# google/neural-light-transport

Hardware: AMD Instinct MI355X
Metric: rendered Mtexels/s at 1024^2 UV (full Model.call forward: U-Net + UV->camera warp); at N > 1: N collective-free replicas of this forward (weak scaling).  The data-parallel TRAIN step with the RCCL gradient all-reduce (BASELINE config 4) is `train_step`: value = Mtexels/s over all ranks, speedup_vs_o (higher is better)
Workload: dtype f32 via 3xbf16 split, 9 exact products, fp32 accumulate (the LDS-tiled encoder convs: fp32 operands as three bf16 terms on v_mfma_f32_16x16x32_bf16, every term product exact in fp32); f32 storage everywhere, every other launch native f32; 1 GPU; BASELINE config 3: dragon_specular relight+view-synth, depth0 16/depth 256, 4 frames/GPU, 1024^2 UV, k=4 obs maps, 512^2 camera warp; frames_per_gpu=4, uv=1024, k=4, cam=512, conv_algo=auto, plan=fused ends, launch=eager, two HIP streams, distinct_batches_rotated=3, launch_tape_replays=0, parallelism=dp1 (frames sharded, no forward collective), world=1, dist_world_size=1, device=cuda:0

## Files before the change

include/nlt_hip.h:

```cpp
#ifndef NLT_HIP_H_
#define NLT_HIP_H_

#ifdef __cplusplus
extern "C" {
#endif

typedef enum {
  NLT_OK = 0,
  NLT_ERR_BAD_ARG = -1,
  NLT_ERR_UNSUPPORTED = -2,
  NLT_ERR_LAUNCH = -3
} nlt_status;

typedef enum {
  NLT_CONV1X1 = 0,
  NLT_CONV_K2S2 = 1,
  NLT_CONV_K2S1 = 2,
  NLT_DECONV_K2S2 = 3,
  NLT_DECONV_K2S1 = 4,
  NLT_CONV_K3S1 = 5,
  NLT_CONV_K3S2 = 6,
  NLT_DECONV_K3S1 = 7,
  NLT_DECONV_K3S2 = 8
} nlt_conv_mode;
// ... 361 lines not shown
int nlt_conv_wino_forward(int mode, const float* src, int ld, int cin, int frames, int kobs, int h, int w,
                          const float* packed, const float* bias, int cout, int tn,
                          float* out, int ldo, float* mean_out, int ldm, int act, float alpha, void* stream);
int nlt_pack_conv_wino_weights_adjoint(int adj_mode, const float* w_keras, int cpre, int cout, int tn, int full, int lo,
                                       float* packed, void* stream);
int nlt_conv_wino_backward_data(int adj_mode, const float* dpre, int ldp, int cpre, int n, int h, int w,
                                const float* packed, int cout, int tn, float* out, int ldo,
                                const float* mask_src, int ldm, float mask_alpha, int accumulate, void* stream);

int nlt_conv_c32_supported(int mode, int cin, int cout);
int nlt_conv_c32_forward(int mode, const float* src, int ld, int cin, int frames, int kobs, int h, int w,
                         const float* packed, const float* bias, int cout,
                         float* out, int ldo, float* mean_out, int ldm, int act, float alpha, void* stream);

long nlt_conv_tile_packed_floats(int mode, int cin, int cout, int tn);
int nlt_pack_conv_tile_weights(int mode, const float* w_keras, int cin, int cout, int tn, float* packed, void* stream);
int nlt_conv_tile_forward(int mode, const float* src, int ld, int cin, int frames, int kobs, int h, int w,
                          const float* packed, const float* bias, int cout, int tn,
                          float* out, int ldo, float* mean_out, int ldm, int act, float alpha, void* stream);

int nlt_pack_conv_tile_weights_adjoint(int adj_mode, const float* w_keras, int cpre, int cout, int tn, int full, int lo,
                                       float* packed, void* stream);
int nlt_conv_tile_backward_data(int adj_mode, const float* dpre, int ldp, int cpre, int n, int h, int w,
                                const float* packed, int cout, int tn, float* out, int ldo,
                                const float* mask_src, int ldm, float mask_alpha, int accumulate,
                                int split_c, const float* split_y, float* split_d, float split_alpha, int split_partial,
                                void* stream);

long nlt_conv_tile3_packed_elems(int mode, int cin, int cout, int tn);
int nlt_pack_conv_tile3_weights(int mode, const float* w_keras, int cin, int cout, int tn, unsigned short* packed, void* stream);
int nlt_conv_tile3_forward(int mode, int nprod, const float* src, int ld, int cin, int frames, int kobs, int h, int w,
                           const unsigned short* packed, const float* bias, int cout, int tn,
                           float* out, int ldo, float* mean_out, int ldm, int act, float alpha, void* stream);

long nlt_chmix_bf16_packed_elems(int cin, int cout);
int nlt_chmix_bf16_pack(const float* w_keras, int cin, int cout, unsigned short* packed, void* stream);
int nlt_chmix_bf16_forward(const unsigned short* x, long texels, int cin, const unsigned short* packed,
                           const float* bias, int cout, int act, float alpha, unsigned short* out, void* stream);

int nlt_conv_k3_forward(int mode, int algo, const float* x, int n, int h, int w, int cin,
                        const float* w_keras, const float* bias, int cout, float* y,
                        int act, float alpha, void* stream);

int nlt_conv_k3_backward_data(int mode, int algo, const float* dpre, int n, int h, int w, int cin,
                              const float* w_keras, int cout, float* dx, void* stream);

long nlt_conv_k3_wgrad_workspace_floats(int mode, int n, int h, int w, int cin, int cout);
int nlt_conv_k3_backward_weights(int mode, const float* x, int n, int h, int w, int cin,
                                 const float* dpre, int cout, float* dw_keras, float* dbias,
                                 float* workspace, long workspace_floats, void* stream);

#ifdef __cplusplus
}
#endif
#endif
```

neural-light-transport_amd/_capi.py:

```python
import ctypes
import threading
import os

import torch

_HERE = os.path.dirname(os.path.abspath(__file__))
LIB_PATH = os.environ.get('NLT_HIP_LIB') or os.path.join(_HERE, 'libnlt_hip.so')

CONV1X1, CONV_K2S2, CONV_K2S1, DECONV_K2S2, DECONV_K2S1 = range(5)
CONV_K3S1, CONV_K3S2, DECONV_K3S1, DECONV_K3S2 = range(5, 9)
ALGO_AUTO, ALGO_DIRECT, ALGO_MFMA = range(3)

_c_int, _c_long, _c_float, _vp = ctypes.c_int, ctypes.c_long, ctypes.c_float, ctypes.c_void_p
_c_double = ctypes.c_double
MAP_F64, MAP_F32, MAP_F16 = range(3)

SIGNATURES = {
    'nlt_version': (ctypes.c_char_p, []),
    'nlt_status_string': (ctypes.c_char_p, [_c_int]),
    'nlt_packed_weight_floats': (_c_long, [_c_int] * 4),
    'nlt_pack_conv_weights': (_c_int, [_c_int, _vp, _c_int, _c_int, _c_int, _vp, _vp]),
    'nlt_conv_forward': (_c_int, [_c_int, _c_int, _c_int, _vp, _c_int, _c_int, _vp, _c_int, _c_int,
                                  _c_int, _c_int, _c_int, _vp, _vp, _vp, _c_int, _vp, _c_int,
                                  _c_int, _c_float, _vp, _c_int, _c_int, _vp]),
# ... 74 lines not shown
    'nlt_conv_forward_splitk': (_c_int, [_c_int, _c_int, _c_int, _vp, _vp, _c_int, _c_int, _vp, _c_int, _c_int,
                                         _c_int, _c_int, _c_int, _vp, _vp, _c_int, _vp, _c_int, _c_int, _c_float,
                                         _vp, _c_int, _c_int, _vp]),
    'nlt_conv_forward_map': (_c_int, [_c_int, _c_int, _c_int, _vp, _vp, _c_int, _c_int, _vp, _c_int, _c_int,
                                      _c_int, _c_int, _c_int, _vp, _vp, _c_int, _vp, _c_int, _c_int, _c_float,
                                      _vp, _c_int, _vp]),
    'nlt_dec_block_forward_map': (_c_int, [_vp, _vp, _c_int, _c_int, _c_int, _c_int, _vp, _vp, _vp, _c_int, _c_float, _vp, _vp, _vp]),
    'nlt_back_forward_map': (_c_int, [_vp, _vp, _c_int, _vp, _c_int, _c_int, _c_int, _vp, _vp, _vp, _vp, _c_float, _vp, _vp, _vp]),
    'nlt_front_ovr_forward': (_c_int, [_vp] * 3 + [_c_int] * 3 + [_vp] * 5 + [_c_int, _c_float, _vp, _c_int, _vp, _vp, _vp]),
    'nlt_front_ovr_forward_u8': (_c_int, [_vp] * 4 + [_c_int] * 3 + [_vp] * 5 + [_c_int, _c_float, _vp, _c_int, _vp, _vp, _vp]),
    'nlt_conv_backward_data': (_c_int, [_c_int, _c_int, _c_int, _vp, _vp, _c_int, _c_int, _c_int, _c_int, _c_int, _vp, _vp, _c_int,
                                        _vp, _c_int, _vp, _c_int, _c_float, _c_int, _c_int, _vp, _vp, _c_float, _c_int, _vp]),
    'nlt_conv_tile_packed_floats': (_c_long, [_c_int] * 4),
    'nlt_pack_conv_tile_weights': (_c_int, [_c_int, _vp, _c_int, _c_int, _c_int, _vp, _vp]),
    'nlt_conv_tile_forward': (_c_int, [_c_int, _vp, _c_int, _c_int, _c_int, _c_int, _c_int, _c_int, _vp, _vp, _c_int, _c_int,
                                       _vp, _c_int, _vp, _c_int, _c_int, _c_float, _vp]),
    'nlt_pack_conv_tile_weights_adjoint': (_c_int, [_c_int, _vp, _c_int, _c_int, _c_int, _c_int, _c_int, _vp, _vp]),
    'nlt_conv_c32_supported': (_c_int, [_c_int] * 3),
    'nlt_conv_c32_forward': (_c_int, [_c_int, _vp, _c_int, _c_int, _c_int, _c_int, _c_int, _c_int, _vp, _vp, _c_int,
                                      _vp, _c_int, _vp, _c_int, _c_int, _c_float, _vp]),
    'nlt_conv_wino_packed_floats': (_c_long, [_c_int] * 4),
    'nlt_pack_conv_wino_weights': (_c_int, [_c_int, _vp, _c_int, _c_int, _c_int, _vp, _vp]),
    'nlt_conv_wino_forward': (_c_int, [_c_int, _vp, _c_int, _c_int, _c_int, _c_int, _c_int, _c_int, _vp, _vp, _c_int, _c_int,
                                       _vp, _c_int, _vp, _c_int, _c_int, _c_float, _vp]),
    'nlt_pack_conv_wino_weights_adjoint': (_c_int, [_c_int, _vp, _c_int, _c_int, _c_int, _c_int, _c_int, _vp, _vp]),
    'nlt_conv_wino_backward_data': (_c_int, [_c_int, _vp, _c_int, _c_int, _c_int, _c_int, _c_int, _vp, _c_int, _c_int, _vp, _c_int,
                                             _vp, _c_int, _c_float, _c_int, _vp]),
    'nlt_conv_tile_backward_data': (_c_int, [_c_int, _vp, _c_int, _c_int, _c_int, _c_int, _c_int, _vp, _c_int, _c_int, _vp, _c_int,
                                             _vp, _c_int, _c_float, _c_int, _c_int, _vp, _vp, _c_float, _c_int, _vp]),
    'nlt_conv_tile3_packed_elems': (_c_long, [_c_int] * 4),
    'nlt_pack_conv_tile3_weights': (_c_int, [_c_int, _vp, _c_int, _c_int, _c_int, _vp, _vp]),
    'nlt_conv_tile3_forward': (_c_int, [_c_int, _c_int, _vp, _c_int, _c_int, _c_int, _c_int, _c_int, _c_int, _vp, _vp, _c_int, _c_int,
                                        _vp, _c_int, _vp, _c_int, _c_int, _c_float, _vp]),
    'nlt_conv_bf16_packed_elems': (_c_long, [_c_int] * 4),
    'nlt_conv_bf16_pack': (_c_int, [_c_int, _vp, _c_int, _c_int, _c_int, _vp, _vp]),
    'nlt_conv_bf16_forward': (_c_int, [_c_int, _c_int, _vp, _c_int, _c_int, _c_int, _vp, _c_int, _c_int, _c_int,
                                       _c_int, _c_int, _c_int, _vp, _vp, _c_int, _vp, _c_int, _c_int, _c_int, _c_float, _vp]),
    'nlt_obs_mean_bf16': (_c_int, [_vp, _c_int, _c_int, _c_long, _c_int, _vp, _c_int, _vp]),
    'nlt_chmix_bf16_packed_elems': (_c_long, [_c_int, _c_int]),
    'nlt_chmix_bf16_pack': (_c_int, [_vp, _c_int, _c_int, _vp, _vp]),
    'nlt_chmix_bf16_forward': (_c_int, [_vp, _c_long, _c_int, _vp, _vp, _c_int, _c_int, _c_float, _vp, _vp]),
    'nlt_cosine_map': (_c_int, [_vp] * 4 + [_c_double] * 3 + [_c_long, _vp, _vp, _vp]),
    'nlt_albedo': (_c_int, [_vp, _c_int, _c_long, _vp, _vp, _vp]),
    'nlt_diffuse_base': (_c_int, [_vp, _vp, _c_int, _c_long, _vp, _vp]),
    'nlt_remap_bilinear_u8': (_c_int, [_vp, _c_int, _c_int, _c_int, _vp, _c_int, _c_int, _c_int, _c_int, _c_int, _vp, _vp]),
    'nlt_remap_bilinear_f32': (_c_int, [_vp, _c_int, _c_int, _c_int, _vp, _c_int, _c_int, _c_int, _c_int, _c_int, _vp, _vp]),
    'nlt_uv_index_map_workspace_bytes': (_c_long, [_c_int, _c_int, _c_long]),
    'nlt_uv_index_map': (_c_int, [_vp, _vp, _c_long, _c_int, _c_int, _c_int, _c_int, _c_double, _vp, _vp, _vp, _vp]),
    'nlt_knn_indices': (_c_int, [_vp, _c_int, _vp, _c_int, _c_int, _vp, _vp]),
    'nlt_psnr_sums': (_c_int, [_vp, _vp, _vp, _c_long, _c_int, _vp, _vp, _vp]),
    'nlt_gather_frames_u8': (_c_int, [_vp, _vp, _c_int, _c_long, _vp, _vp]),
    'nlt_assemble_batch': (_c_int, [_vp] * 6 + [_c_int, _c_int, _c_long, _c_int] + [_vp] * 6 + [_vp]),
    'nlt_warp_backward_det_workspace_bytes': (_c_long, [_c_int] * 5),
    'nlt_warp_backward_det': (_c_int, [_vp, _vp] + [_c_int] * 5 + [_vp, _vp, _c_long, _vp]),
    'nlt_resize_bilinear_backward_gather': (_c_int, [_vp] + [_c_int] * 6 + [_vp, _vp]),
    'nlt_loss_det_workspace_floats': (_c_long, [_c_int]),
    'nlt_l2_loss_forward_det': (_c_int, [_vp, _vp, _c_int, _c_long, _vp, _vp, _c_long, _vp]),
    'nlt_l2_loss_weighted_forward_det': (_c_int, [_vp, _vp, _vp, _c_int, _c_long, _c_int, _vp, _vp, _c_long, _vp]),
    'nlt_l2_train_loss_det': (_c_int, [_vp, _vp, _vp, _c_int, _c_long, _c_float, _vp, _vp, _vp, _vp, _c_long, _vp]),
    'nlt_barron_det_slots_floats': (_c_long, [_c_int] * 3),
    'nlt_barron_loss_det': (_c_int, [_vp, _vp, _c_int, _c_int, _c_int, _vp, _vp, _vp, _vp, _c_long, _vp]),
    'nlt_stem_backward_det_workspace_floats': (_c_long, [_c_int] * 4),
    'nlt_stem_backward_det': (_c_int, [_vp] * 6 + [_c_int] * 5 + [_vp] * 6 + [_vp, _c_long, _vp]),
    'nlt_head_backward_det_workspace_floats': (_c_long, [_c_int] * 5),
    'nlt_head_backward_det': (_c_int, [_vp, _c_int, _c_int, _vp, _c_int, _c_int, _vp, _vp, _c_int, _c_int, _c_int,
                                       _vp, _c_int, _vp, _c_int, _vp, _vp, _vp, _c_long, _vp]),
# ... 819 lines not shown


def pack_conv_wino_weights(mode, w_keras, cin, cout, tn, full=None, lo=0):
    src = (mode, _ptr(_dense(w_keras, 'w_keras')), cin, cout, tn)
    if full is None:
        name, args = 'nlt_pack_conv_wino_weights', src
    else:
        name, args = 'nlt_pack_conv_wino_weights_adjoint', src + (full, lo)
    return _pack('nlt_conv_wino_packed_floats', (mode, cin, cout, tn), name, args, torch.float32, w_keras.device)


def conv_wino_forward(mode, src, ld, cin, frames, kobs, h, w, packed, bias, cout, tn, out, ldo, mean_out, ldm, act=True, alpha=0.3):
    _call('nlt_conv_wino_forward', mode, _ptr(src), ld, cin, frames, kobs, h, w, _ptr(packed), _ptr(bias), cout, tn, _ptr(out), ldo,
          _ptr(mean_out), ldm, 1 if act else 0, float(alpha))


def conv_wino_backward_data(adj_mode, dpre, cpre, ldp, n, h, w, packed, cout, tn, out, ldo, mask_src=None, ldm=0, mask_alpha=0.3,
                            accumulate=False):
    _call('nlt_conv_wino_backward_data', adj_mode, _ptr(dpre), ldp, cpre, n, h, w, _ptr(packed), cout, tn, _ptr(out), ldo,
          _ptr(mask_src), ldm, float(mask_alpha), 1 if accumulate else 0)


def pack_conv_tile3_weights(mode, w_keras, cin, cout, tn):
    return _pack('nlt_conv_tile3_packed_elems', (mode, cin, cout, tn),
                 'nlt_pack_conv_tile3_weights', (mode, _ptr(_dense(w_keras, 'w_keras')), cin, cout, tn), torch.int16, w_keras.device)


def conv_tile3_forward(mode, src, ld, cin, frames, kobs, h, w, packed, bias, cout, tn, out, ldo, mean_out, ldm,
                       act=True, alpha=0.3, nprod=6):
    _call('nlt_conv_tile3_forward', mode, nprod, _ptr(src), ld, cin, frames, kobs, h, w, packed.data_ptr(), _ptr(bias), cout, tn,
          _ptr(out), ldo, _ptr(mean_out), ldm, 1 if act else 0, float(alpha))


def conv_bf16_pack(mode, w_keras, c0, c1, cout):
    return _pack('nlt_conv_bf16_packed_elems', (mode, c0, c1, cout),
                 'nlt_conv_bf16_pack', (mode, _ptr(_dense(w_keras, 'w_keras')), c0, c1, cout), torch.bfloat16, w_keras.device)


def _any_ptr(t, what):
    if t is None:
        return None, 0
    if not (t.is_cuda and t.dtype in (torch.float32, torch.bfloat16)):
        raise NLTError("%s: expected a float32 / bfloat16 CUDA tensor, got %s on %s" % (what, t.dtype, t.device))
    return t.data_ptr(), 1 if t.dtype == torch.float32 else 0


def conv_bf16_forward(mode, src0, c0, ld0, src1, c1, ld1, n, h, w, w_packed, bias, cout, out, ldo, act=True, alpha=0.3, tile_hint=0):
    p0, f0 = _any_ptr(src0, 'src0')
    p1, f1 = _any_ptr(src1, 'src1')
    po, fo = _any_ptr(out, 'out')
    _call('nlt_conv_bf16_forward', mode, tile_hint, p0, ld0, c0, f0, p1, ld1, c1, f1, n, h, w,
          _tptr(w_packed, torch.bfloat16, 'w_packed'), _ptr(bias), cout, po, ldo, fo, 1 if act else 0, float(alpha))


def obs_mean_bf16(obs, n, k, hw, c, out, ldo):
    if obs.dtype != torch.bfloat16 or out.dtype != torch.bfloat16:
        raise NLTError("obs_mean_bf16: bfloat16 tensors expected")
    _call('nlt_obs_mean_bf16', obs.data_ptr(), n, k, hw, c, out.data_ptr(), ldo)


def chmix_bf16_pack(w_keras):
    cin, cout = w_keras.shape[2], w_keras.shape[3]
    return _pack('nlt_chmix_bf16_packed_elems', (cin, cout),
                 'nlt_chmix_bf16_pack', (_ptr(_dense(w_keras, 'w_keras')), cin, cout), torch.bfloat16, w_keras.device)


# ... 245 lines not shown
```

neural-light-transport_amd/csrc/conv_tile3.hip:

```cpp
#include "nlt_common.h"
#include "pack_common.h"

namespace {

typedef __attribute__((ext_vector_type(8))) __bf16 bf16x8;
typedef unsigned short u16;
typedef unsigned int u32x4 __attribute__((ext_vector_type(4)));

constexpr int TH = 8, TW = 16;
constexpr int QS2 = 272, ODD2 = 132;
constexpr int PL = 160;

template <int MODE> struct T3;
template <> struct T3<NLT_CONV_K2S1> { static constexpr int PAIRS = 2, B_UNITS = 153 * 2, B_SLOTS = 6 * PL; };
template <> struct T3<NLT_CONV_K2S2> { static constexpr int PAIRS = 1, B_UNITS = 256 * 2, B_SLOTS = 6 * QS2; };

struct Tile3P {
  const float* src; const u16* packed; const float* bias;
  float* out; float* mean_out;
  int ld, cin, frames, kobs, h, w;
  int oh, ow, cout, ldo, ldm;
  int tiles_y, tiles_x, ncc;
  int act; float alpha;
};
// ... 205 lines not shown
              const f32x4 bv = *reinterpret_cast<const f32x4*>(p.bias + oc);
#pragma unroll
              for (int rt = 0; rt < RT; ++rt) {
                const int gy = ty0 + wm * RT + rt, gx = tx0 + j;
                f32x4 v = acc[e][rt][ct] + bv;
                if (p.act) {
#pragma unroll
                  for (int c4 = 0; c4 < 4; ++c4) v[c4] = v[c4] > 0.f ? v[c4] : p.alpha * v[c4];
                }
                acc[e][rt][ct] = (f32x4){0.f, 0.f, 0.f, 0.f};
                mean[rt][ct] += v;
                if (gy < p.oh && gx < p.ow) {
                  const long ot = ((long)(f * p.kobs + i) * p.oh + gy) * p.ow + gx;
                  if (p.out) *reinterpret_cast<f32x4*>(p.out + ot * p.ldo + oc) = v;
                  if (p.mean_out && i == p.kobs - 1) {
                    const long mt = ((long)f * p.oh + gy) * p.ow + gx;
                    *reinterpret_cast<f32x4*>(p.mean_out + mt * p.ldm + oc) = mean[rt][ct] * (1.f / (float)p.kobs);
                  }
                }
              }
            }
          }
        }
        if (more) {
          if (new_slab) store_a(sa ^ 1);
          store_b((q + 1) & 1);
        }
        __syncthreads();
      }
    }
  }
}

template <int MODE, int TNT, int KO>
int launch3k(const Tile3P& p, int nprod, hipStream_t s) {
  const long tiles = (long)p.frames * p.tiles_y * p.tiles_x;
  const dim3 grid((unsigned)tiles, (unsigned)(p.cout / (16 * TNT)));
  if (nprod == 9) hipLaunchKernelGGL((conv_tile3_kernel<MODE, TNT, 9, KO>), grid, dim3(256), 0, s, p);
  else if (nprod == 6) hipLaunchKernelGGL((conv_tile3_kernel<MODE, TNT, 6, KO>), grid, dim3(256), 0, s, p);
  else if (KO > 1) return NLT_ERR_UNSUPPORTED;
  else if (nprod == 3) hipLaunchKernelGGL((conv_tile3_kernel<MODE, TNT, 3, 1>), grid, dim3(256), 0, s, p);
  else hipLaunchKernelGGL((conv_tile3_kernel<MODE, TNT, 1, 1>), grid, dim3(256), 0, s, p);
  NLT_CHECK_LAUNCH();
  return NLT_OK;
}

template <int MODE, int TNT>
int launch3(const Tile3P& p, int nprod, hipStream_t s) {
  static const int want = [] { const char* e = getenv("NLT_TILE3_KO"); return e ? atoi(e) : 0; }();
  const int cap = want > 0 ? want : (TNT == 2 ? 4 : (MODE == NLT_CONV_K2S1 ? 1 : 2));
  if (nprod >= 6) {
    if (TNT == 2 && cap >= 4 && p.kobs % 4 == 0) return launch3k<MODE, TNT, (TNT == 2 ? 4 : 1)>(p, nprod, s);
    if (cap >= 2 && p.kobs % 2 == 0) return launch3k<MODE, TNT, 2>(p, nprod, s);
  }
  return launch3k<MODE, TNT, 1>(p, nprod, s);
}

}

extern "C" long nlt_conv_tile3_packed_elems(int mode, int cin, int cout, int tn) {
  if ((mode != NLT_CONV_K2S1 && mode != NLT_CONV_K2S2) || cin <= 0 || cout <= 0) return -1;
  if ((cin & 15) || (tn != 32 && tn != 64) || cout % tn) return -1;
  return (long)12 * cin * cout;
}

extern "C" int nlt_pack_conv_tile3_weights(int mode, const float* w_keras, int cin, int cout, int tn, unsigned short* packed,
                                           void* stream) {
  const long total = nlt_conv_tile3_packed_elems(mode, cin, cout, tn);
  if (total <= 0) return NLT_ERR_UNSUPPORTED;
  if (!w_keras || !packed || !nlt_aligned16(packed)) return NLT_ERR_BAD_ARG;
  hipLaunchKernelGGL(pack_tile3_kernel, dim3((unsigned)((total + 255) / 256)), dim3(256), 0, static_cast<hipStream_t>(stream),
                     w_keras, cin, cout, tn / 16, total, packed);
  NLT_CHECK_LAUNCH();
  return NLT_OK;
}

extern "C" int nlt_conv_tile3_forward(int mode, int nprod, const float* src, int ld, int cin, int frames, int kobs, int h, int w,
                                      const unsigned short* packed, const float* bias, int cout, int tn,
                                      float* out, int ldo, float* mean_out, int ldm, int act, float alpha, void* stream) {
  if (!src || !packed || !bias || (!out && !mean_out) || (nprod != 1 && nprod != 3 && nprod != 6 && nprod != 9)) return NLT_ERR_BAD_ARG;
  if (frames <= 0 || kobs <= 0 || h <= 0 || w <= 0 || cin <= 0 || cout <= 0) return NLT_ERR_BAD_ARG;
  if (nlt_conv_tile3_packed_elems(mode, cin, cout, tn) <= 0) return NLT_ERR_UNSUPPORTED;
  if (mode == NLT_CONV_K2S2 && ((h | w) & 1)) return NLT_ERR_UNSUPPORTED;
  if (ld < cin || (ld & 3) || (out && (ldo < cout || (ldo & 3))) || (mean_out && (ldm < cout || (ldm & 3)))) return NLT_ERR_BAD_ARG;
  if (!nlt_aligned16(src) || !nlt_aligned16(packed) || !nlt_aligned16(bias) || (out && !nlt_aligned16(out)) ||
      (mean_out && !nlt_aligned16(mean_out))) return NLT_ERR_BAD_ARG;
  if ((long long)frames * kobs * h * w * (long long)(ld > ldo ? ld : ldo) >= (1ll << 31)) return NLT_ERR_UNSUPPORTED;
  Tile3P p;
  p.src = src; p.packed = packed; p.bias = bias; p.out = out; p.mean_out = mean_out;
  p.ld = ld; p.cin = cin; p.frames = frames; p.kobs = kobs; p.h = h; p.w = w;
  p.oh = mode == NLT_CONV_K2S2 ? h / 2 : h; p.ow = mode == NLT_CONV_K2S2 ? w / 2 : w;
  p.cout = cout; p.ldo = ldo; p.ldm = ldm; p.ncc = cin / 16; p.act = act; p.alpha = alpha;
  p.tiles_y = (p.oh + TH - 1) / TH; p.tiles_x = (p.ow + TW - 1) / TW;
  hipStream_t s = static_cast<hipStream_t>(stream);
  if (mode == NLT_CONV_K2S1) return tn == 64 ? launch3<NLT_CONV_K2S1, 4>(p, nprod, s) : launch3<NLT_CONV_K2S1, 2>(p, nprod, s);
  return tn == 64 ? launch3<NLT_CONV_K2S2, 4>(p, nprod, s) : launch3<NLT_CONV_K2S2, 2>(p, nprod, s);
}
```

neural-light-transport_amd/engine.py:

```python
import os

import torch

from . import _capi as C
from .engine_infer import OverrideMixin


class OpTimer:

    def __init__(self):
        self.pending, self.records = [], {}
        self.flops = {}
        self.moved = {}

    def launch(self, label, nbytes, fn, *args, **kw):
        e0, e1 = torch.cuda.Event(enable_timing=True), torch.cuda.Event(enable_timing=True)
        e0.record()
        fn(*args, **kw)
        e1.record()
        self.pending.append((label, nbytes, e0, e1))

    def collect(self):
        torch.cuda.synchronize()
        for label, nbytes, e0, e1 in self.pending:
# ... 199 lines not shown
            return False
        if kobs == 1 and mean_out is None:
            if self._trial_wino >> 8:
                return False
            unfold = False
        self._enc_launch(C.conv_wino_forward, layer.packed_wino(tn), (tn,), self._ran_wino, unfold, label, layer, act, src, cin, ld,
                         frames, kobs, h, w, out, ldo, mean_out, ldm)
        return True

    def _conv_bf(self, label, layer, act, src0, c0, ld0, src1, c1, ld1, n, h, w, out, ldo):
        layer.build(c0 + c1, src0.device)
        assert layer.cin == c0 + c1, (layer.cin, c0, c1)
        oh, ow = layer.out_hw(h, w)
        bpe = lambda t: 4 if t.dtype == torch.float32 else 2
        moved = n * h * w * (c0 * bpe(src0) + (c1 * bpe(src1) if c1 else 0)) + n * oh * ow * layer.n_ch_out * bpe(out)
        self._launch(label, 4 * (n * h * w * (c0 + c1) + n * oh * ow * layer.n_ch_out), C.conv_bf16_forward, layer.mode,
                     src0, c0, ld0, src1, c1, ld1, n, h, w, layer.packed_bf16(c0, c1), layer.bias.detach(), layer.n_ch_out, out, ldo,
                     **_act_kw(act), tile_hint=self.tile_hints.get('bf.' + label, 0),
                     flops=_gemm(layer.mode, n, h, w, c0 + c1, layer.n_ch_out)[2], moved=moved)

    def _conv_enc(self, label, layer, act, src, cin, ld, frames, kobs, h, w, out, ldo, algo, mean_out=None, ldm=0,
                  obs_weights=None):
        layer.build(cin, src.device)
        conv = (label, layer, act, src, cin, ld, frames, kobs, h, w, out, ldo, mean_out, ldm)
        chint = self._trial_c32 or self.c32_hints.get(label, 0)
        if (chint and self.use_c32 and algo == C.ALGO_AUTO and obs_weights is None and layer.cin == cin and ld % 4 == 0 and ldo % 4 == 0
                and C.conv_c32_supported(layer.mode, cin, layer.n_ch_out) and not (chint == 2 and kobs == 1 and self._trial_c32)):
            self._enc_launch(C.conv_c32_forward, layer.packed_tile(32), (), self._ran_c32, chint == 2 and kobs > 1, *conv)
            return
        if (algo == C.ALGO_AUTO and layer.mode == C.CONV_K2S1 and (self._trial_wino or label in self.wino_hints)
                and self._wino(*conv, obs_weights)):
            return
        hint = self._trial_lds or (0 if (self._trial_wino or self._trial_c32) else self.lds_hints.get(label, 0))
        tn, unfold = hint & 255, bool(hint >> 8)
        ok = (tn and obs_weights is None and algo == C.ALGO_AUTO and layer.mode in (C.CONV_K2S2, C.CONV_K2S1)
              and layer.cin == cin and cin % 16 == 0 and layer.n_ch_out % tn == 0)
        if ok and unfold and kobs == 1:
            ok = self._trial_lds == 0
            unfold = False
        if ok and self.precision in ('f32x3', 'f32x3_9'):
            self._enc_launch(C.conv_tile3_forward, layer.packed_tile3(tn), (tn,), self._ran_lds, unfold, *conv,
                             nprod=9 if self.precision == 'f32x3_9' else 6)
        elif ok:
            self._enc_launch(C.conv_tile_forward, layer.packed_tile(tn), (tn,), self._ran_lds, unfold, *conv)
        else:
            self._conv(label, layer, act, src, cin, ld, None, 0, 0, frames * kobs, h, w, out, ldo, algo)
            if mean_out is not None:
                oh, ow = layer.out_hw(h, w)
                self._mean(label, out, obs_weights, frames, kobs, oh * ow, layer.n_ch_out, mean_out, ldm)

    def _dec_block_plain(self, b, j, lab, da, dact_a, db, dact_b, srcs, n, hh, ww, algo, s2_label=None, bmap=None):
        nl = da.n_ch_out
        self._conv(s2_label or lab + '.s2', da, dact_a, *srcs, n, hh, ww, b['dtmp'][j], nl, algo, bmap=bmap)
        self._conv(lab + '.s1', db, dact_b, b['dtmp'][j], nl, nl, None, 0, 0, n, 2 * hh, 2 * ww, b['dec'][j], db.n_ch_out, algo)
        return b['dec'][j], db.n_ch_out

    def _autotune(self, run, backward=False):
        saved = (self.timer, dict(self.tile_hints), dict(self.algo_hints))
        self._tuning = True
        results = {}
        trials = [('tile', 16 * r + c) for r in (1, 2, 4) for c in (1, 2, 4)]
        if not self.fuse_ends and not backward:
            trials.append(('direct', 0))
        if not backward:
            trials += [('lds', 32), ('lds', 64), ('lds', 256 + 32), ('lds', 256 + 64)]
        elif self.tile_dgrad:
            trials += [('lds', 32), ('lds', 64)]
        if self.use_c32 and not backward:
            trials += [('c32', 1), ('c32', 2)]
        if self.use_wino:
            trials += [('wino', 32), ('wino', 64)] + ([('wino', 256 + 32), ('wino', 256 + 64)] if not backward else [])
        mode = os.environ.get('NLT_SPLITK', 'all')
        if mode == 'all' or (mode == 'fwd' and not backward):
            forms = os.environ.get('NLT_SPLITK_FORMS', 'both')
            cand = ((4, 8, 16, 32, 64, 128) if forms != 'two' else ()) + ((-16, -32, -64, -128) if forms == 'both' else ()) + \
                   ((-4, -8, -16, -32, -64, -128) if forms == 'two' else ())
            trials += [('splitk', (16 * r + c, ks)) for (r, c) in ((1, 1), (1, 2), (2, 2), (1, 4)) for ks in cand]
        saved_lds, saved_sk, saved_wino, saved_c32 = dict(self.lds_hints), dict(self.splitk_hints), dict(self.wino_hints), dict(self.c32_hints)
        for kind, hint in trials:
            self.tile_hints = {'*': hint} if kind == 'tile' else ({'*': hint[0]} if kind == 'splitk' else {})
            self.algo_hints = {}
            self.lds_hints, self.splitk_hints, self.wino_hints, self.c32_hints = {}, {}, {}, {}
            self._trial_direct = kind == 'direct'
            self._trial_lds = hint if kind == 'lds' else 0
            self._trial_wino = hint if kind == 'wino' else 0
            self._trial_c32 = hint if kind == 'c32' else 0
            self._trial_splitk = hint[1] if kind == 'splitk' else 0
            self._ran_direct, self._ran_lds, self._ran_splitk, self._ran_wino, self._ran_c32 = set(), set(), set(), set(), set()
            self.timer = None
            run()
            self.timer = OpTimer()
            run(); run()
            rec = self.timer.collect()
            for label, r in rec.items():
                t = r[1] / r[0]
                if label.endswith('.o.s1') and label.replace('.s1', '.mean') in rec:
                    m = rec[label.replace('.s1', '.mean')]
                    t += m[1] / m[0]
# ... 708 lines not shown
```

Before: 3540 Mtexels/s.

## Add persistent resident-workgroup tile3 conv kernels with LDS-held weights and autotune hints

Adds persistent variants of the 3xbf16 LDS-tiled encoder convolution. Each workgroup stays resident, keeps the packed weights for its output-channel group in LDS (up to 160 KB), and loops over a contiguous range of tiles with double-buffered input staging. For K2S1 with tn=32, a per-wave variant uses only wave-level barriers. The autotuner gains new 'lds' hints (512+tn) that select this path, so it runs only when tuning prefers it. The aim is to stop re-reading weights per tile and to cut launch and tail overhead, at the cost of occupancy and a larger dynamic-LDS request.

```diff
diff --git a/include/nlt_hip.h b/include/nlt_hip.h
--- a/include/nlt_hip.h
+++ b/include/nlt_hip.h
@@ -417,6 +417,9 @@
 int nlt_conv_tile3_forward(int mode, int nprod, const float* src, int ld, int cin, int frames, int kobs, int h, int w,
                            const unsigned short* packed, const float* bias, int cout, int tn,
                            float* out, int ldo, float* mean_out, int ldm, int act, float alpha, void* stream);
+int nlt_conv_tile3r_forward(int mode, int nprod, const float* src, int ld, int cin, int frames, int kobs, int h, int w,
+                            const unsigned short* packed, const float* bias, int cout, int tn,
+                            float* out, int ldo, float* mean_out, int ldm, int act, float alpha, int max_workgroups, void* stream);
 
 long nlt_chmix_bf16_packed_elems(int cin, int cout);
 int nlt_chmix_bf16_pack(const float* w_keras, int cin, int cout, unsigned short* packed, void* stream);
diff --git a/neural-light-transport_amd/_capi.py b/neural-light-transport_amd/_capi.py
--- a/neural-light-transport_amd/_capi.py
+++ b/neural-light-transport_amd/_capi.py
@@ -130,6 +130,8 @@
     'nlt_pack_conv_tile3_weights': (_c_int, [_c_int, _vp, _c_int, _c_int, _c_int, _vp, _vp]),
     'nlt_conv_tile3_forward': (_c_int, [_c_int, _c_int, _vp, _c_int, _c_int, _c_int, _c_int, _c_int, _c_int, _vp, _vp, _c_int, _c_int,
                                         _vp, _c_int, _vp, _c_int, _c_int, _c_float, _vp]),
+    'nlt_conv_tile3r_forward': (_c_int, [_c_int, _c_int, _vp, _c_int, _c_int, _c_int, _c_int, _c_int, _c_int, _vp, _vp, _c_int, _c_int,
+                                         _vp, _c_int, _vp, _c_int, _c_int, _c_float, _c_int, _vp]),
     'nlt_conv_bf16_packed_elems': (_c_long, [_c_int] * 4),
     'nlt_conv_bf16_pack': (_c_int, [_c_int, _vp, _c_int, _c_int, _c_int, _vp, _vp]),
     'nlt_conv_bf16_forward': (_c_int, [_c_int, _c_int, _vp, _c_int, _c_int, _c_int, _vp, _c_int, _c_int, _c_int,
@@ -1015,6 +1017,26 @@
           _ptr(out), ldo, _ptr(mean_out), ldm, 1 if act else 0, float(alpha))
 
 
+def conv_tile3r_plan(mode, cin, tn):
+    if mode not in (CONV_K2S1, CONV_K2S2) or cin % 16 or tn not in (32, 64):
+        return None
+    if mode == CONV_K2S1 and tn == 32:
+        for rows in (4, 2):
+            lds = cin * 768 + 8 * 6 * (((rows + 1) * 17 + 15) // 16 * 16) * 16
+            if lds <= 160 * 1024:
+                return (lds, 8, 1, rows)
+    lds = cin * (tn // 16) * 384 + 2 * 6 * (160 if mode == CONV_K2S1 else 272) * 16
+    if lds > 160 * 1024:
+        return None
+    return (lds, 8, 1, 8) if 2 * lds > 160 * 1024 else (lds, 4, 2, 8)
+
+
+def conv_tile3r_forward(mode, src, ld, cin, frames, kobs, h, w, packed, bias, cout, tn, out, ldo, mean_out, ldm,
+                        act=True, alpha=0.3, nprod=6, max_workgroups=0):
+    _call('nlt_conv_tile3r_forward', mode, nprod, _ptr(src), ld, cin, frames, kobs, h, w, packed.data_ptr(), _ptr(bias), cout, tn,
+          _ptr(out), ldo, _ptr(mean_out), ldm, 1 if act else 0, float(alpha), max_workgroups)
+
+
 def conv_bf16_pack(mode, w_keras, c0, c1, cout):
     return _pack('nlt_conv_bf16_packed_elems', (mode, c0, c1, cout),
                  'nlt_conv_bf16_pack', (mode, _ptr(_dense(w_keras, 'w_keras')), c0, c1, cout), torch.bfloat16, w_keras.device)
diff --git a/neural-light-transport_amd/csrc/conv_tile3.hip b/neural-light-transport_amd/csrc/conv_tile3.hip
--- a/neural-light-transport_amd/csrc/conv_tile3.hip
+++ b/neural-light-transport_amd/csrc/conv_tile3.hip
@@ -261,8 +261,450 @@
   }
 }
 
+extern __shared__ u32x4 tile3r_lds[];
+
+template <int MODE, int TNT, int NPROD, int KO, int NWV>
+__global__ __launch_bounds__(64 * NWV, 2) void conv_tile3r_kernel(Tile3P p, int ngroups) {
+  using TT = T3<MODE>;
+  constexpr int NT = 64 * NWV;
+  constexpr int WN = TNT == 4 ? 2 : 1, WM = NWV / WN, RT = TH / WM, CT = 2;
+  constexpr int A_SLOTS = TT::PAIRS * TNT * 3 * 64;
+  constexpr int NB = (TT::B_UNITS + NT - 1) / NT;
+  constexpr int BPL = MODE == NLT_CONV_K2S1 ? PL : QS2;
+  const int a_group = p.ncc * 2 * TNT * 3 * 64;
+  u32x4* const lds_b = tile3r_lds + a_group;
+
+  const int tid = threadIdx.x, lane = tid & 63, wave = tid >> 6;
+  const int kk = lane >> 4, j = lane & 15;
+  const int wn = wave % WN, wm = wave / WN;
+  const int spf = (MODE == NLT_CONV_K2S1 ? 1 : 2) * p.ncc;
+  const int groups = p.kobs / KO;
+  const long in_frame = (long)p.h * p.w;
+  const int tiles = p.frames * p.tiles_y * p.tiles_x;
+  const long items = (long)tiles * ngroups;
+  const int rank = xcd_tile3(blockIdx.x, gridDim.x);
+  int it = (int)(rank * items / gridDim.x);
+  const int it_end = (int)((rank + 1) * items / gridDim.x);
+  if (it >= it_end) return;
+
+  int b_lds[NB], b_hf[NB]; long b_tex[NB]; bool b_ok[NB], b_st[NB];
+#pragma unroll
+  for (int i = 0; i < NB; ++i) {
+    const int u = tid + NT * i;
+    const int hf = (u >> 3) & 1, tx = (u >> 4) * 8 + (u & 7);
+    b_hf[i] = hf;
+    if (MODE == NLT_CONV_K2S1) {
+      b_st[i] = tx < 153;
+      b_lds[i] = hf * PL + tx;
+    } else {
+      const int y = tx >> 5, xx = tx & 31;
+      b_st[i] = tx < 256;
+      b_lds[i] = hf * QS2 + (xx & 1) * ODD2 + y * 16 + (xx >> 1);
+    }
+  }
+  int ng = 0, nf = 0, nty0 = 0, ntx0 = 0;
+  auto geom = [&](int item) {
+    ng = item / tiles;
+    int t = item - ng * tiles;
+    ntx0 = (t % p.tiles_x) * TW; t /= p.tiles_x;
+    nty0 = (t % p.tiles_y) * TH;
+    nf = t / p.tiles_y;
+#pragma unroll
+    for (int i = 0; i < NB; ++i) {
+      const int u = tid + NT * i;
+      const int tx = (u >> 4) * 8 + (u & 7);
+      if (MODE == NLT_CONV_K2S1) {
+        const int gy = nty0 + tx / 17, gx = ntx0 + tx % 17;
+        b_ok[i] = b_st[i] && gy < p.h && gx < p.w;
+        b_tex[i] = (long)gy * p.w + gx;
+      } else {
+        const int y = tx >> 5, xx = tx & 31;
+        const int gy = 2 * (nty0 + y), gx = 2 * ntx0 + xx;
+        b_ok[i] = b_st[i] && (nty0 + y) < p.oh && gx < p.w;
+        b_tex[i] = (long)gy * p.w + gx;
+      }
+    }
+  };
+
+  f32x4 rb[NB][2];
+  auto load_b = [&](int s, int frame) {
+    const int cc = MODE == NLT_CONV_K2S1 ? s : (s >> 1);
+    const int a = MODE == NLT_CONV_K2S1 ? 0 : (s & 1);
+    const float* sp = p.src + ((long)(nf * p.kobs + frame) * in_frame + (long)a * p.w) * p.ld + cc * 16;
+#pragma unroll
+    for (int n = 0; n < NB; ++n) {
+      const float* q8 = sp + (b_ok[n] ? b_tex[n] : 0) * p.ld + 8 * b_hf[n];
+      const f32x4 v0 = *reinterpret_cast<const f32x4*>(q8), v1 = *reinterpret_cast<const f32x4*>(q8 + 4);
+      const f32x4 z = {0.f, 0.f, 0.f, 0.f};
+      rb[n][0] = b_ok[n] ? v0 : z;
+      rb[n][1] = b_ok[n] ? v1 : z;
+    }
+  };
+  auto store_b = [&](int buf) {
+    u32x4* base = lds_b + buf * TT::B_SLOTS;
+#pragma unroll
+    for (int n = 0; n < NB; ++n) {
+      if (!b_st[n]) continue;
+      unsigned hi[4], mid[4], lo[4];
+      split2(rb[n][0][0], rb[n][0][1], hi[0], mid[0], lo[0]);
+      split2(rb[n][0][2], rb[n][0][3], hi[1], mid[1], lo[1]);
+      split2(rb[n][1][0], rb[n][1][1], hi[2], mid[2], lo[2]);
+      split2(rb[n][1][2], rb[n][1][3], hi[3], mid[3], lo[3]);
+      u32x4* bb = base + b_lds[n];
+      bb[0] = (u32x4){hi[0], hi[1], hi[2], hi[3]};
+      bb[2 * BPL] = (u32x4){mid[0], mid[1], mid[2], mid[3]};
+      bb[4 * BPL] = (u32x4){lo[0], lo[1], lo[2], lo[3]};
+    }
+  };
+  auto copy_a = [&](int grp) {
+    const u32x4* ap = reinterpret_cast<const u32x4*>(p.packed) + (long)grp * a_group;
+    for (int i = tid; i < a_group; i += NT) tile3r_lds[i] = ap[i];
+  };
+
+  f32x4 acc[KO][RT][CT], mean[RT][CT];
+#pragma unroll
+  for (int rt = 0; rt < RT; ++rt)
+#pragma unroll
+    for (int ct = 0; ct < CT; ++ct) {
+      mean[rt][ct] = (f32x4){0.f, 0.f, 0.f, 0.f};
+#pragma unroll
+      for (int io = 0; io < KO; ++io) acc[io][rt][ct] = mean[rt][ct];
+    }
+
+  geom(it);
+  load_b(0, 0);
+  copy_a(ng);
+  store_b(0);
+  __syncthreads();
+  int q = 0;
+  for (; it < it_end; ++it) {
+    const int g = ng, f = nf, ty0 = nty0, tx0 = ntx0;
+    const bool last_item = it + 1 == it_end;
+    for (int gi = 0; gi < groups; ++gi) {
+      for (int s = 0; s < spf; ++s) {
+#pragma unroll
+        for (int io = 0; io < KO; ++io, ++q) {
+          const bool new_slab = io + 1 == KO;
+          int ns = s, ngi = gi;
+          if (new_slab) { if (++ns == spf) { ns = 0; ++ngi; } }
+          const bool item_end = ngi == groups;
+          if (item_end) {
+            ngi = 0;
+            if (!last_item) geom(it + 1);
+          }
+          load_b(ns, ngi * KO + (new_slab ? 0 : io + 1));
+          const u32x4* A = tile3r_lds + s * A_SLOTS;
+          const u32x4* B = lds_b + (q & 1) * TT::B_SLOTS;
+#pragma unroll
+          for (int pl = 0; pl < TT::PAIRS; ++pl) {
+            bf16x8 bt[3][RT], at[3][CT];
+#pragma unroll
+            for (int rt = 0; rt < RT; ++rt) {
+              const int y = wm * RT + rt;
+              const int slot = MODE == NLT_CONV_K2S1 ? (kk & 1) * PL + (y + pl) * 17 + j + (kk >> 1)
+                                                     : (kk & 1) * QS2 + (kk >> 1) * ODD2 + y * 16 + j;
+#pragma unroll
+              for (int t = 0; t < 3; ++t) bt[t][rt] = __builtin_bit_cast(bf16x8, B[t * 2 * BPL + slot]);
+            }
+#pragma unroll
+            for (int ct = 0; ct < CT; ++ct)
+#pragma unroll
+              for (int t = 0; t < 3; ++t)
+                at[t][ct] = __builtin_bit_cast(bf16x8, A[((pl * TNT + wn * CT + ct) * 3 + t) * 64 + lane]);
+            constexpr int ORDER9[9][2] = {{2, 2}, {2, 1}, {1, 2}, {2, 0}, {0, 2}, {1, 1}, {1, 0}, {0, 1}, {0, 0}};
+#pragma unroll
+            for (int pi = 9 - NPROD; pi < 9; ++pi)
+#pragma unroll
+              for (int rt = 0; rt < RT; ++rt)
+#pragma unroll
+                for (int ct = 0; ct < CT; ++ct)
+                  acc[io][rt][ct] = __builtin_amdgcn_mfma_f32_16x16x32_bf16(at[ORDER9[pi][0]][ct], bt[ORDER9[pi][1]][rt], acc[io][rt][ct], 0, 0, 0);
+          }
+          if (s == spf - 1 && io == KO - 1) {
+#pragma unroll
+            for (int e = 0; e < KO; ++e) {
+              const int i = gi * KO + e;
+#pragma unroll
+              for (int ct = 0; ct < CT; ++ct) {
+                const int oc = (g * TNT + wn * CT + ct) * 16 + 4 * kk;
+                const f32x4 bv = *reinterpret_cast<const f32x4*>(p.bias + oc);
+#pragma unroll
+                for (int rt = 0; rt < RT; ++rt) {
+                  const int gy = ty0 + wm * RT + rt, gx = tx0 + j;
+                  f32x4 v = acc[e][rt][ct] + bv;
+                  if (p.act) {
+#pragma unroll
+                    for (int c4 = 0; c4 < 4; ++c4) v[c4] = v[c4] > 0.f ? v[c4] : p.alpha * v[c4];
+                  }
+                  acc[e][rt][ct] = (f32x4){0.f, 0.f, 0.f, 0.f};
+                  mean[rt][ct] += v;
+                  if (gy < p.oh && gx < p.ow) {
+                    const long ot = ((long)(f * p.kobs + i) * p.oh + gy) * p.ow + gx;
+                    if (p.out) *reinterpret_cast<f32x4*>(p.out + ot * p.ldo + oc) = v;
+                    if (p.mean_out && i == p.kobs - 1) {
+                      const long mt = ((long)f * p.oh + gy) * p.ow + gx;
+                      *reinterpret_cast<f32x4*>(p.mean_out + mt * p.ldm + oc) = mean[rt][ct] * (1.f / (float)p.kobs);
+                    }
+                  }
+                  if (i == p.kobs - 1) mean[rt][ct] = (f32x4){0.f, 0.f, 0.f, 0.f};
+                }
+              }
+            }
+          }
+          if (!(item_end && last_item)) store_b((q + 1) & 1);
+          __syncthreads();
+        }
+      }
+    }
+    if (!last_item && ng != g) {
+      copy_a(ng);
+      __syncthreads();
+    }
+  }
+}
+
+constexpr size_t TILE3R_LDS_CU = 160 * 1024;
+
+int tile3r_cus() {
+  static const int n = [] {
+    int dev = 0, v = 0;
+    if (hipGetDevice(&dev) != hipSuccess) return 0;
+    if (hipDeviceGetAttribute(&v, hipDeviceAttributeMultiprocessorCount, dev) != hipSuccess) return 0;
+    return v;
+  }();
+  return n;
+}
+
+int tile3r_allow_lds(const void* kernel, size_t lds, size_t (&done)[8]) {
+  int dev = 0;
+  if (lds <= 64 * 1024) return NLT_OK;
+  if (hipGetDevice(&dev) != hipSuccess) return NLT_ERR_LAUNCH;
+  if (dev >= 0 && dev < 8 && done[dev] >= lds) return NLT_OK;
+  if (hipFuncSetAttribute(kernel, hipFuncAttributeMaxDynamicSharedMemorySize, (int)lds) != hipSuccess) return NLT_ERR_LAUNCH;
+  if (dev >= 0 && dev < 8) done[dev] = lds;
+  return NLT_OK;
+}
+
+template <int MODE, int TNT, int NPROD, int KO, int NWV>
+int launch3r_k(const Tile3P& p, size_t lds, int nwg, hipStream_t s) {
+  auto* k = conv_tile3r_kernel<MODE, TNT, NPROD, KO, NWV>;
+  static size_t done[8] = {};
+  if (tile3r_allow_lds(reinterpret_cast<const void*>(k), lds, done) != NLT_OK) return NLT_ERR_LAUNCH;
+  hipLaunchKernelGGL(k, dim3((unsigned)nwg), dim3(64 * NWV), lds, s, p, p.cout / (16 * TNT));
+  NLT_CHECK_LAUNCH();
+  return NLT_OK;
+}
+
+template <int RT, int NPROD>
+__global__ __launch_bounds__(512, 2) void conv_tile3w_kernel(Tile3P p, int ngroups, int tiles_y) {
+  constexpr int TNT = 2, CT = 2, NWV = 8;
+  constexpr int ROWS = RT + 1, UNITS = ROWS * 17 * 2, NB = (UNITS + 63) / 64;
+  constexpr int PLW = (ROWS * 17 + 15) / 16 * 16;
+  constexpr int A_SLOTS = 2 * TNT * 3 * 64;
+  const int a_group = p.ncc * A_SLOTS;
+  const int tid = threadIdx.x, lane = tid & 63, wave = tid >> 6;
+  const int kk = lane >> 4, j = lane & 15;
+  u32x4* const B = tile3r_lds + a_group + wave * (6 * PLW);
+  const long in_frame = (long)p.h * p.w;
+  const int tiles = p.frames * tiles_y * p.tiles_x;
+  const long items = (long)tiles * ngroups;
+  const int rank = xcd_tile3(blockIdx.x, gridDim.x);
+  const int it0 = (int)(rank * items / gridDim.x), it1 = (int)((rank + 1) * items / gridDim.x);
+
+  int b_lds[NB], b_hf[NB], b_tx[NB]; long b_tex[NB]; bool b_ok[NB], b_st[NB];
+#pragma unroll
+  for (int i = 0; i < NB; ++i) {
+    const int u = lane + 64 * i;
+    b_hf[i] = (u >> 3) & 1;
+    b_tx[i] = (u >> 4) * 8 + (u & 7);
+    b_st[i] = b_tx[i] < ROWS * 17;
+    b_lds[i] = b_hf[i] * PLW + b_tx[i];
+  }
+  int nf = 0, nty0 = 0, ntx0 = 0;
+  auto geom = [&](int t) {
+    ntx0 = (t % p.tiles_x) * TW; t /= p.tiles_x;
+    nty0 = (t % tiles_y) * RT;
+    nf = t / tiles_y;
+#pragma unroll
+    for (int i = 0; i < NB; ++i) {
+      const int gy = nty0 + b_tx[i] / 17, gx = ntx0 + b_tx[i] % 17;
+      b_ok[i] = b_st[i] && gy < p.h && gx < p.w;
+      b_tex[i] = (long)gy * p.w + gx;
+    }
+  };
+  f32x4 rb[NB][2];
+  auto load_b = [&](int cc, int frame) {
+    const float* sp = p.src + (long)(nf * p.kobs + frame) * in_frame * p.ld + cc * 16;
+#pragma unroll
+    for (int n = 0; n < NB; ++n) {
+      const float* q8 = sp + (b_ok[n] ? b_tex[n] : 0) * p.ld + 8 * b_hf[n];
+      const f32x4 v0 = *reinterpret_cast<const f32x4*>(q8), v1 = *reinterpret_cast<const f32x4*>(q8 + 4);
+      const f32x4 z = {0.f, 0.f, 0.f, 0.f};
+      rb[n][0] = b_ok[n] ? v0 : z;
+      rb[n][1] = b_ok[n] ? v1 : z;
+    }
+  };
+  auto store_b = [&]() {
+#pragma unroll
+    for (int n = 0; n < NB; ++n) {
+      if (!b_st[n]) continue;
+      unsigned hi[4], mid[4], lo[4];
+      split2(rb[n][0][0], rb[n][0][1], hi[0], mid[0], lo[0]);
+      split2(rb[n][0][2], rb[n][0][3], hi[1], mid[1], lo[1]);
+      split2(rb[n][1][0], rb[n][1][1], hi[2], mid[2], lo[2]);
+      split2(rb[n][1][2], rb[n][1][3], hi[3], mid[3], lo[3]);
+      u32x4* bb = B + b_lds[n];
+      bb[0] = (u32x4){hi[0], hi[1], hi[2], hi[3]};
+      bb[2 * PLW] = (u32x4){mid[0], mid[1], mid[2], mid[3]};
+      bb[4 * PLW] = (u32x4){lo[0], lo[1], lo[2], lo[3]};
+    }
+  };
+  auto wave_sync = [&]() {
+    __builtin_amdgcn_fence(__ATOMIC_RELEASE, "wavefront");
+    __builtin_amdgcn_wave_barrier();
+    __builtin_amdgcn_fence(__ATOMIC_ACQUIRE, "wavefront");
+  };
+
+  int seg = it0;
+  while (seg < it1) {
+    const int g = seg / tiles;
+    const int seg_end = min(it1, (g + 1) * tiles);
+    {
+      const u32x4* ap = reinterpret_cast<const u32x4*>(p.packed) + (long)g * a_group;
+      for (int i = tid; i < a_group; i += 64 * NWV) tile3r_lds[i] = ap[i];
+    }
+    __syncthreads();
+    int it = seg + wave;
+    if (it < seg_end) {
+      f32x4 acc[RT][CT], mean[RT][CT];
+#pragma unroll
+      for (int rt = 0; rt < RT; ++rt)
+#pragma unroll
+        for (int ct = 0; ct < CT; ++ct) acc[rt][ct] = mean[rt][ct] = (f32x4){0.f, 0.f, 0.f, 0.f};
+      geom(it - g * tiles);
+      load_b(0, 0);
+      store_b();
+      wave_sync();
+      for (; it < seg_end; it += NWV) {
+        const int f = nf, ty0 = nty0, tx0 = ntx0;
+        const bool last_item = it + NWV >= seg_end;
+        for (int i = 0; i < p.kobs; ++i) {
+          for (int s = 0; s < p.ncc; ++s) {
+            int ns = s + 1, ni = i;
+            if (ns == p.ncc) { ns = 0; ++ni; }
+            const bool item_end = ni == p.kobs;
+            if (item_end) {
+              ni = 0;
+              if (!last_item) geom(it + NWV - g * tiles);
+            }
+            load_b(ns, ni);
+            bf16x8 bt[3][ROWS];
+#pragma unroll
+            for (int r = 0; r < ROWS; ++r)
+#pragma unroll
+              for (int t = 0; t < 3; ++t)
+                bt[t][r] = __builtin_bit_cast(bf16x8, B[t * 2 * PLW + (kk & 1) * PLW + r * 17 + j + (kk >> 1)]);
+            wave_sync();
+            const u32x4* A = tile3r_lds + s * A_SLOTS;
+#pragma unroll
+            for (int pl = 0; pl < 2; ++pl) {
+              bf16x8 at[3][CT];
+#pragma unroll
+              for (int ct = 0; ct < CT; ++ct)
+#pragma unroll
+                for (int t = 0; t < 3; ++t) at[t][ct] = __builtin_bit_cast(bf16x8, A[((pl * TNT + ct) * 3 + t) * 64 + lane]);
+              constexpr int ORDER9[9][2] = {{2, 2}, {2, 1}, {1, 2}, {2, 0}, {0, 2}, {1, 1}, {1, 0}, {0, 1}, {0, 0}};
+#pragma unroll
+              for (int pi = 9 - NPROD; pi < 9; ++pi)
+#pragma unroll
+                for (int rt = 0; rt < RT; ++rt)
+#pragma unroll
+                  for (int ct = 0; ct < CT; ++ct)
+                    acc[rt][ct] = __builtin_amdgcn_mfma_f32_16x16x32_bf16(at[ORDER9[pi][0]][ct], bt[ORDER9[pi][1]][rt + pl], acc[rt][ct], 0, 0, 0);
+            }
+            if (!(item_end && last_item)) store_b();
+            wave_sync();
+            if (s == p.ncc - 1) {
+#pragma unroll
+              for (int ct = 0; ct < CT; ++ct) {
+                const int oc = (g * TNT + ct) * 16 + 4 * kk;
+                const f32x4 bv = *reinterpret_cast<const f32x4*>(p.bias + oc);
+#pragma unroll
+                for (int rt = 0; rt < RT; ++rt) {
+                  const int gy = ty0 + rt, gx = tx0 + j;
+                  f32x4 v = acc[rt][ct] + bv;
+                  if (p.act) {
+#pragma unroll
+                    for (int c4 = 0; c4 < 4; ++c4) v[c4] = v[c4] > 0.f ? v[c4] : p.alpha * v[c4];
+                  }
+                  acc[rt][ct] = (f32x4){0.f, 0.f, 0.f, 0.f};
+                  mean[rt][ct] += v;
+                  if (gy < p.oh && gx < p.ow) {
+                    const long ot = ((long)(f * p.kobs + i) * p.oh + gy) * p.ow + gx;
+                    if (p.out) *reinterpret_cast<f32x4*>(p.out + ot * p.ldo + oc) = v;
+                    if (p.mean_out && i == p.kobs - 1) {
+                      const long mt = ((long)f * p.oh + gy) * p.ow + gx;
+                      *reinterpret_cast<f32x4*>(p.mean_out + mt * p.ldm + oc) = mean[rt][ct] * (1.f / (float)p.kobs);
+                    }
+                  }
+                  if (i == p.kobs - 1) mean[rt][ct] = (f32x4){0.f, 0.f, 0.f, 0.f};
+                }
+              }
+            }
+          }
+        }
+      }
+    }
+    seg = seg_end;
+    if (seg < it1) __syncthreads();
+  }
+}
+
+template <int RT>
+int launch3w(const Tile3P& p, int nprod, int max_wg, hipStream_t s) {
+  constexpr int PLW = ((RT + 1) * 17 + 15) / 16 * 16;
+  const size_t lds = (size_t)p.cin * 2 * 384 + 8 * 6 * PLW * sizeof(u32x4);
+  if (lds > TILE3R_LDS_CU) return NLT_ERR_UNSUPPORTED;
+  const int cus = tile3r_cus();
+  if (cus <= 0) return NLT_ERR_LAUNCH;
+  const int tiles_y = (p.oh + RT - 1) / RT;
+  const long items = (long)p.frames * tiles_y * p.tiles_x * (p.cout / 32);
+  long nwg = cus;
+  if (max_wg > 0 && nwg > max_wg) nwg = max_wg;
+  if (nwg > items) nwg = items;
+  auto* k = nprod == 9 ? conv_tile3w_kernel<RT, 9> : conv_tile3w_kernel<RT, 6>;
+  static size_t done[2][8] = {};
+  if (tile3r_allow_lds(reinterpret_cast<const void*>(k), lds, done[nprod == 9]) != NLT_OK) return NLT_ERR_LAUNCH;
+  hipLaunchKernelGGL(k, dim3((unsigned)nwg), dim3(512), lds, s, p, p.cout / 32, tiles_y);
+  NLT_CHECK_LAUNCH();
+  return NLT_OK;
+}
+
 template <int MODE, int TNT, int KO>
-int launch3k(const Tile3P& p, int nprod, hipStream_t s) {
+int launch3r(const Tile3P& p, int nprod, int max_wg, hipStream_t s) {
+  if (nprod != 6 && nprod != 9) return NLT_ERR_UNSUPPORTED;
+  if (MODE == NLT_CONV_K2S1 && TNT == 2) {
+    int st = launch3w<4>(p, nprod, max_wg, s);
+    if (st == NLT_ERR_UNSUPPORTED) st = launch3w<2>(p, nprod, max_wg, s);
+    if (st != NLT_ERR_UNSUPPORTED) return st;
+  }
+  const size_t lds = (size_t)p.cin * TNT * 384 + 2 * T3<MODE>::B_SLOTS * sizeof(u32x4);
+  if (lds > TILE3R_LDS_CU) return NLT_ERR_UNSUPPORTED;
+  const bool wide = 2 * lds > TILE3R_LDS_CU;
+  const int cus = tile3r_cus();
+  if (cus <= 0) return NLT_ERR_LAUNCH;
+  const long items = (long)p.frames * p.tiles_y * p.tiles_x * (p.cout / (16 * TNT));
+  long nwg = (long)cus * (wide ? 1 : 2);
+  if (max_wg > 0 && nwg > max_wg) nwg = max_wg;
+  if (nwg > items) nwg = items;
+  if (items >= (1l << 31)) return NLT_ERR_UNSUPPORTED;
+  if (wide) return nprod == 9 ? launch3r_k<MODE, TNT, 9, KO, 8>(p, lds, (int)nwg, s) : launch3r_k<MODE, TNT, 6, KO, 8>(p, lds, (int)nwg, s);
+  return nprod == 9 ? launch3r_k<MODE, TNT, 9, KO, 4>(p, lds, (int)nwg, s) : launch3r_k<MODE, TNT, 6, KO, 4>(p, lds, (int)nwg, s);
+}
+
+template <int MODE, int TNT, int KO>
+int launch3k(const Tile3P& p, int nprod, hipStream_t s, int resident_wg) {
+  if (resident_wg >= 0) return launch3r<MODE, TNT, KO>(p, nprod, resident_wg, s);
   const long tiles = (long)p.frames * p.tiles_y * p.tiles_x;
   const dim3 grid((unsigned)tiles, (unsigned)(p.cout / (16 * TNT)));
   if (nprod == 9) hipLaunchKernelGGL((conv_tile3_kernel<MODE, TNT, 9, KO>), grid, dim3(256), 0, s, p);
@@ -275,14 +717,14 @@
 }
 
 template <int MODE, int TNT>
-int launch3(const Tile3P& p, int nprod, hipStream_t s) {
+int launch3(const Tile3P& p, int nprod, hipStream_t s, int resident_wg) {
   static const int want = [] { const char* e = getenv("NLT_TILE3_KO"); return e ? atoi(e) : 0; }();
-  const int cap = want > 0 ? want : (TNT == 2 ? 4 : (MODE == NLT_CONV_K2S1 ? 1 : 2));
+  const int cap = want > 0 ? want : (TNT == 2 ? 4 : (MODE == NLT_CONV_K2S1 || resident_wg >= 0 ? 1 : 2));
   if (nprod >= 6) {
-    if (TNT == 2 && cap >= 4 && p.kobs % 4 == 0) return launch3k<MODE, TNT, (TNT == 2 ? 4 : 1)>(p, nprod, s);
-    if (cap >= 2 && p.kobs % 2 == 0) return launch3k<MODE, TNT, 2>(p, nprod, s);
+    if (TNT == 2 && cap >= 4 && p.kobs % 4 == 0) return launch3k<MODE, TNT, (TNT == 2 ? 4 : 1)>(p, nprod, s, resident_wg);
+    if (cap >= 2 && p.kobs % 2 == 0) return launch3k<MODE, TNT, 2>(p, nprod, s, resident_wg);
   }
-  return launch3k<MODE, TNT, 1>(p, nprod, s);
+  return launch3k<MODE, TNT, 1>(p, nprod, s, resident_wg);
 }
 
 }
@@ -304,9 +746,9 @@
   return NLT_OK;
 }
 
-extern "C" int nlt_conv_tile3_forward(int mode, int nprod, const float* src, int ld, int cin, int frames, int kobs, int h, int w,
-                                      const unsigned short* packed, const float* bias, int cout, int tn,
-                                      float* out, int ldo, float* mean_out, int ldm, int act, float alpha, void* stream) {
+static int tile3_forward(int mode, int nprod, const float* src, int ld, int cin, int frames, int kobs, int h, int w,
+                         const unsigned short* packed, const float* bias, int cout, int tn,
+                         float* out, int ldo, float* mean_out, int ldm, int act, float alpha, int resident_wg, void* stream) {
   if (!src || !packed || !bias || (!out && !mean_out) || (nprod != 1 && nprod != 3 && nprod != 6 && nprod != 9)) return NLT_ERR_BAD_ARG;
   if (frames <= 0 || kobs <= 0 || h <= 0 || w <= 0 || cin <= 0 || cout <= 0) return NLT_ERR_BAD_ARG;
   if (nlt_conv_tile3_packed_elems(mode, cin, cout, tn) <= 0) return NLT_ERR_UNSUPPORTED;
@@ -322,6 +764,23 @@
   p.cout = cout; p.ldo = ldo; p.ldm = ldm; p.ncc = cin / 16; p.act = act; p.alpha = alpha;
   p.tiles_y = (p.oh + TH - 1) / TH; p.tiles_x = (p.ow + TW - 1) / TW;
   hipStream_t s = static_cast<hipStream_t>(stream);
-  if (mode == NLT_CONV_K2S1) return tn == 64 ? launch3<NLT_CONV_K2S1, 4>(p, nprod, s) : launch3<NLT_CONV_K2S1, 2>(p, nprod, s);
-  return tn == 64 ? launch3<NLT_CONV_K2S2, 4>(p, nprod, s) : launch3<NLT_CONV_K2S2, 2>(p, nprod, s);
-}
+  if (mode == NLT_CONV_K2S1)
+    return tn == 64 ? launch3<NLT_CONV_K2S1, 4>(p, nprod, s, resident_wg) : launch3<NLT_CONV_K2S1, 2>(p, nprod, s, resident_wg);
+  return tn == 64 ? launch3<NLT_CONV_K2S2, 4>(p, nprod, s, resident_wg) : launch3<NLT_CONV_K2S2, 2>(p, nprod, s, resident_wg);
+}
+
+extern "C" int nlt_conv_tile3_forward(int mode, int nprod, const float* src, int ld, int cin, int frames, int kobs, int h, int w,
+                                      const unsigned short* packed, const float* bias, int cout, int tn,
+                                      float* out, int ldo, float* mean_out, int ldm, int act, float alpha, void* stream) {
+  return tile3_forward(mode, nprod, src, ld, cin, frames, kobs, h, w, packed, bias, cout, tn, out, ldo, mean_out, ldm, act, alpha,
+                       -1, stream);
+}
+
+extern "C" int nlt_conv_tile3r_forward(int mode, int nprod, const float* src, int ld, int cin, int frames, int kobs, int h, int w,
+                                       const unsigned short* packed, const float* bias, int cout, int tn,
+                                       float* out, int ldo, float* mean_out, int ldm, int act, float alpha, int max_workgroups,
+                                       void* stream) {
+  if (max_workgroups < 0) return NLT_ERR_BAD_ARG;
+  return tile3_forward(mode, nprod, src, ld, cin, frames, kobs, h, w, packed, bias, cout, tn, out, ldo, mean_out, ldm, act, alpha,
+                       max_workgroups, stream);
+}
diff --git a/neural-light-transport_amd/engine.py b/neural-light-transport_amd/engine.py
--- a/neural-light-transport_amd/engine.py
+++ b/neural-light-transport_amd/engine.py
@@ -255,15 +255,19 @@
                 and self._wino(*conv, obs_weights)):
             return
         hint = self._trial_lds or (0 if (self._trial_wino or self._trial_c32) else self.lds_hints.get(label, 0))
-        tn, unfold = hint & 255, bool(hint >> 8)
+        tn, unfold = hint & 255, bool((hint >> 8) & 1)
+        resident = bool(hint & 512)
         ok = (tn and obs_weights is None and algo == C.ALGO_AUTO and layer.mode in (C.CONV_K2S2, C.CONV_K2S1)
               and layer.cin == cin and cin % 16 == 0 and layer.n_ch_out % tn == 0)
+        if ok and resident and (self.precision not in ('f32x3', 'f32x3_9') or C.conv_tile3r_plan(layer.mode, cin, tn) is None):
+            ok = self._trial_lds == 0
+            resident = False
         if ok and unfold and kobs == 1:
             ok = self._trial_lds == 0
             unfold = False
         if ok and self.precision in ('f32x3', 'f32x3_9'):
-            self._enc_launch(C.conv_tile3_forward, layer.packed_tile3(tn), (tn,), self._ran_lds, unfold, *conv,
-                             nprod=9 if self.precision == 'f32x3_9' else 6)
+            self._enc_launch(C.conv_tile3r_forward if resident else C.conv_tile3_forward, layer.packed_tile3(tn), (tn,),
+                             self._ran_lds, unfold, *conv, nprod=9 if self.precision == 'f32x3_9' else 6)
         elif ok:
             self._enc_launch(C.conv_tile_forward, layer.packed_tile(tn), (tn,), self._ran_lds, unfold, *conv)
         else:
@@ -287,6 +291,8 @@
             trials.append(('direct', 0))
         if not backward:
             trials += [('lds', 32), ('lds', 64), ('lds', 256 + 32), ('lds', 256 + 64)]
+            if self.precision in ('f32x3', 'f32x3_9'):
+                trials += [('lds', 512 + 32), ('lds', 512 + 64)]
         elif self.tile_dgrad:
             trials += [('lds', 32), ('lds', 64)]
         if self.use_c32 and not backward:
```

New measurement: 3671 Mtexels/s (median of 6 runs). +3.7%, better.
